# lijun9250lj/video-steganography-PCAMV

Measured on AMD Instinct MI355X. Metric: 1080p macroblocks/s (embed on), higher is better.
Workload: dtype u8

## Files before the change

### video-steganography-pcamv_amd/csrc/pcamv_common.h

```cpp
#ifndef PCAMV_COMMON_H
#define PCAMV_COMMON_H
#include <stddef.h>
#include <stdint.h>
#include "../../include/pcamv_gpu.h"

#ifdef PCAMV_HOST_EMU
#define PCAMV_DEV static inline
#define PCAMV_CONST static const
#else
#include <hip/hip_runtime.h>
#define PCAMV_DEV __device__ __forceinline__
#define PCAMV_CONST __device__ static const
#endif

#define PCAMV_PAD 32
#define PCAMV_CPAD 16
#define PCAMV_LSW 28
#define PCAMV_LROW 32
#define PCAMV_LSTRIPS(stride) (((stride) + PCAMV_LSW - 1) / PCAMV_LSW + 1)
#define PCAMV_LSTRIP_OF(x) (((uint32_t)(x) * 18725u) >> 19)
#define PCAMV_COST_MAX (1 << 28)
#define PCAMV_COST_MV_LEN (4 * 4 * 2048 + 1)
#define PCAMV_COST_MV_CENTRE (2 * 4 * 2048)
#define SCAN8_0 (4 + 1 * 8)
// ... 59 lines not shown
PCAMV_DEV int scan8_of(int idx) { return SCAN8_0 + blk_x_of(idx) + 8 * blk_y_of(idx); }
PCAMV_DEV int clip3i(int v, int lo, int hi) { return v < lo ? lo : v > hi ? hi : v; }
PCAMV_DEV int iabs(int v) { return v < 0 ? -v : v; }
PCAMV_DEV int imin(int a, int b) { return a < b ? a : b; }
PCAMV_DEV int imax(int a, int b) { return a > b ? a : b; }
PCAMV_DEV int median3i(int a, int b, int c) { return imax(imin(a, b), imin(imax(a, b), c)); }
PCAMV_DEV int size_ue_of(unsigned v) { int n = 0; for (v++; v > 1; v >>= 1) n++; return 2 * n + 1; }
enum { I4_V, I4_H, I4_DC, I4_DDL, I4_DDR, I4_VR, I4_HD, I4_VL, I4_HU, I4_DC_LEFT, I4_DC_TOP, I4_DC_128 };

struct MBLocal {
    uint8_t fenc[24 * 16];
    int16_t cmv[48][2];
    int8_t cref[48];
    int16_t pskip_mv[2];
    int16_t mvr_own[2];
    int mb_x, mb_y, mb_xy;
    int mv_min[2], mv_max[2], mv_min_spel[2], mv_max_spel[2], mv_min_fpel[2], mv_max_fpel[2];
    int neighbour, type_left, type_top, type_topleft, type_topright;
    int i_type, i_partition;
    uint8_t sub_part[4];
    int b_skip_mc, cbp_luma, cbp_chroma;
    int nnz_mask;
    uint32_t cxy[64];
    int ccost[192];
    int slots[16];
    uint8_t recb[24 * 16];
    uint8_t recb0[24 * 16];
    uint8_t pred[24 * 16];
    union {
        struct {
            int16_t coef[24][16];
            int16_t cdc[2][4];
            int blk_nz[24], blk_score[24];
            int red[64];
        };
        uint8_t pred4[4][24 * 16];
    };
    int mvc16[9][2];
    int nbc[12];
    uint32_t win[(4 * 480 + 2 * 192) / 4];
    int win_x0, win_y0, win_cx0, win_cy0;
    uint8_t ib_top[3][28];
    uint8_t ib_left[3][16];
    uint8_t nzc[48];
    int16_t cmvd[48][2];
    int8_t i4mode[48];
    int cbp_left, cbp_top;
    int b_fast_intra, fenc_satd_sum, fenc_sa8d_sum;
    uint8_t snap_pred[24 * 16];
    uint8_t snap_nzc[48];
    int16_t snap_cmvd[48][2];
    int snap_cbp_luma, snap_cbp_chroma, snap_nnz_mask;
    int snap_part, snap_cost;
#ifdef PCAMV_SEARCH_CALL
    const struct FrameDev *fdesc;
    int me_tmp[10];
    int mvc_tmp[9][2];
#endif
};
#define PCAMV_PASS2_LDS ((int)offsetof(MBLocal, coef))
static_assert(offsetof(MBLocal, pred) + sizeof(((MBLocal *)0)->pred) == offsetof(MBLocal, coef), "pred must end at the second pass' LDS cut");
static_assert(offsetof(MBLocal, fenc) < PCAMV_PASS2_LDS && offsetof(MBLocal, cmv) < PCAMV_PASS2_LDS && offsetof(MBLocal, cref) < PCAMV_PASS2_LDS &&
              offsetof(MBLocal, nnz_mask) < PCAMV_PASS2_LDS && offsetof(MBLocal, slots) + sizeof(((MBLocal *)0)->slots) <= PCAMV_PASS2_LDS &&
              offsetof(MBLocal, ccost) + sizeof(((MBLocal *)0)->ccost) <= PCAMV_PASS2_LDS, "a field the second pass uses lies beyond its LDS");
static_assert(offsetof(MBLocal, ccost) == offsetof(MBLocal, cxy) + sizeof(((MBLocal *)0)->cxy), "cxy and ccost must be contiguous (cab_residual_walk)");
static_assert(offsetof(MBLocal, recb0) == offsetof(MBLocal, recb) + 384 && offsetof(MBLocal, pred) == offsetof(MBLocal, recb) + 768 &&
              offsetof(MBLocal, coef) == offsetof(MBLocal, recb) + 1152, "recb, recb0, pred, the union must be contiguous in this order (TESA_SLOT, L_IFD)");
#define PCAMV_CHAIN_NZ 464
#define PCAMV_CHAIN_MVD 488
#define PCAMV_CHAIN_BYTES 576
#define L_CAB(L, k) ((uint8_t *)(L)->win + 464 * (k))
#define PCAMV_CAB_USED 276
#define L_CABT(L) ((uint8_t *)(L)->win + 464)
#define L_CABK(L) ((uint8_t *)(L)->win + 464 + PCAMV_CAB_USED)
#define L_CTAB(L) ((L)->win + 256)
#define L_IFD(L) ((uint8_t *)(L)->recb)
#define IFD(L, x, y) (L_IFD(L)[((y) + 1) * 32 + (x) + 4])
PCAMV_DEV int scan8_all_of(int idx)
{
    if (idx < 16) return scan8_of(idx);
    if (idx < 24) return 1 + ((idx - 16) & 1) + 8 * (1 + (((idx - 16) >> 1) & 1) + 3 * ((idx - 16) >> 2));
    return 4 + (idx - 24) + 5 * 8;
}

#define TESA_MAX_RANGE 16
#define TESA_REGION_A ((int)((3 * 24 * 16 + 4 * 24 * 16) / 4))
#define TESA_SLOT(L, i) ((i) < TESA_REGION_A ? (uint32_t *)((uint8_t *)(L) + offsetof(MBLocal, recb)) + (i) : (L)->win + ((i) - TESA_REGION_A))
#define TESA_PACK(sad, ry, rx) ((uint32_t)(sad) << 12 | (uint32_t)(ry) << 6 | (uint32_t)(rx))
#define TESA_SAD(e) ((int)((e) >> 12))
#define NB_LEFT 1
#define NB_TOP 2
#define NB_TOPRIGHT 4
#define NB_TOPLEFT 8

#define CAND_PACK(X, Y) ((uint32_t)(uint16_t)(X) | ((uint32_t)(uint16_t)(Y) << 16))
#define CAND_NONE 0x80008000u
#define CAND_X(c) ((int)(int16_t)(L->cxy[c] & 0xffffu))
#define CAND_Y(c) ((int)(int16_t)(L->cxy[c] >> 16))
#define EV_SATD 1
#define EV_CHROMA 2
#define EV_FPEL 4
#define EV_NOMV 8
#define EV_PROBE 16
#define EV_WIN 32
#define EV_SRC4 64
#define WIN_LW 24
#define WIN_LH 20
#define WIN_LP (WIN_LW * WIN_LH)
#define WIN_CW 16
#define WIN_CH 12
#define WIN_CP (WIN_CW * WIN_CH)
struct EvalRes { int cost, idx; };
#ifdef PCAMV_HOST_EMU
// ... 57 lines not shown
```

### video-steganography-pcamv_amd/csrc/pcamv_kernels.hip.h

```cpp
#ifndef PCAMV_KERNELS_HIP_H
#define PCAMV_KERNELS_HIP_H
#include "pcamv_common.h"
#include "pcamv_prims_gpu.h"
#include "pcamv_mbkernels.h"
#include "stc_mats.h"
#include "pcamv_stc_extract.h"

#if !defined(PCAMV_TESA_TU) && !defined(PCAMV_RD_TU)
#define PCAMV_MAIN_TU 1
#endif

#ifdef PCAMV_MAIN_TU
static __global__ void __launch_bounds__(256) k_chroma_pad(const FrameDev *__restrict__ Fs)
{
    const FrameDev &F = Fs[blockIdx.z >> 1];
    const int pl = blockIdx.z & 1;
    const uint8_t *__restrict__ src = F.raw[1 + pl];
    uint8_t *__restrict__ dst = F.chroma_base[pl];
    const int w = F.w >> 1, h = F.h >> 1, cstride = F.cstride, clines = F.clines;
    const int x = 4 * (blockIdx.x * blockDim.x + threadIdx.x), y = blockIdx.y;
    if (x >= cstride || y >= clines) return;
    const uint8_t *rowp = src + (size_t)clip3i(y - PCAMV_CPAD, 0, h - 1) * w;
    const int gx = x - PCAMV_CPAD;
    uint32_t v;
// ... 643 lines not shown
        const unsigned long long t_f = PROF_T();
        __builtin_amdgcn_fence(__ATOMIC_ACQUIRE, "wavefront");
        const int g = (int)((item - 1u) >> 16), xy = (int)((item - 1u) & 0xffffu);
        const FrameDev F = Fs[g];
        const int y = xy / fl.mb_w, x = xy - y * fl.mb_w;
        if (MODE == 0) PROF_ADD(15, t_f);
        PROF_ADD(MODE ? 13 : 0, t_pop);
        const unsigned long long t_s = PROF_T();
#ifdef PCAMV_SEARCH_CALL
        if (MODE == 0 && lane == 0) L.fdesc = Fs + g;
#endif
        if (MODE == 0 && (TESA & 4)) { if (!mbk_search_spec<TESA>(F, &L, Ap, x, y, fl, g, item)) break; }
        else if (MODE == 0) mbk_search<TESA>(F, &L, Ap, x, y);
        else {
            const int x0 = fl.unit * x, n = imin(fl.unit, F.mb_w - x0);
            p2_unit_load(F, Up, x0, y, n);
            for (int k = 0; k < n; k++) {
                P2Pre pre;
                pre.r = &Up->rec[k]; pre.base = Up->car_base[k]; pre.any_flip = Up->mbflip[k]; pre.nnz1 = Up->nnz1[k]; pre.drain = k > 0;
                if (mbk_pass2(F, &L, x0 + k, y, 0, &pre)) p2_put_mb(Up, &L, k);
                mbk_deblock_unit(F, Up, &L, k, x0 + k, y);
            }
            p2_unit_store(F, Up, x0, y, n);
        }
        PROF_ADD(MODE ? 14 : 1, t_s);
        const unsigned long long t_p = PROF_T();
        asm volatile("s_waitcnt vmcnt(0)" ::: "memory");
        if (MODE == 0 && (TESA & 4)) { }
        else if (lane == 0 && fl.raster) {
            if (xy + 1 < fl.n_mb) flow_done_one(fl, g & (fl.nq - 1), g * fl.n_mb + xy + 1, item + 1u);
        } else if (lane == 0) {
            const int base = g * fl.n_mb, q = g & (fl.nq - 1);
            if (x + 1 < fl.mb_w) flow_done_one(fl, q, base + xy + 1, item + 1u);
            if (y + 1 < fl.mb_h) {
                if (x >= 1) flow_done_one(fl, q, base + xy + fl.mb_w - 1, item + (unsigned)fl.mb_w - 1u);
                if (x == fl.mb_w - 1) flow_done_one(fl, q, base + xy + fl.mb_w, item + (unsigned)fl.mb_w);
            }
        }
        PROF_ADD(MODE ? 15 : 2, t_p);
        const unsigned long long t_r = PROF_T();
        if (MODE == 0 && fl.fused) {
            if (!fl.raster) {
                if (lane == 0) ticket = __hip_atomic_fetch_add(&fl.ctr[FLOW_HEAD(home)], 1u, RLX_AGENT);
                have_ticket = true;
            }
            mbk_rca_encode(F, &L, Ap, xy, 1, (TESA & 2) && F.b_mbrd);
        }
        PROF_ADD(3, t_r);
        if (MODE == 0) PROF_ADD(4, t_pop);
    }
    PROF_FLUSH();
}

#ifdef PCAMV_MAIN_TU
static __global__ void __launch_bounds__(64, PCAMV_FLOW_OCC) k_analyse_flow(const FrameDev *__restrict__ Fs, FlowDev fl)
{
    __shared__ MBLocal L;
    __shared__ Analysis A;
    flow_loop<0, 0>(Fs, fl, L, &A, nullptr);
}
#endif
#ifdef PCAMV_TESA_TU
static __global__ void __launch_bounds__(64, PCAMV_FLOW_OCC) k_analyse_flow_tesa(const FrameDev *__restrict__ Fs, FlowDev fl)
{
    __shared__ MBLocal L;
    __shared__ Analysis A;
    flow_loop<0, 1>(Fs, fl, L, &A, nullptr);
}
#endif
void pcamv_launch_flow_tesa(unsigned waves, hipStream_t st, const FrameDev *dF, const FlowDev &fl);
#ifdef PCAMV_RD_TU
#ifndef PCAMV_RD_OCC
#define PCAMV_RD_OCC 4
#endif
#ifndef PCAMV_RD_VARIANT
#define PCAMV_RD_VARIANT 2
#endif
static __global__ void __launch_bounds__(64, PCAMV_RD_OCC) k_analyse_flow_rd(const FrameDev *__restrict__ Fs, FlowDev fl)
{
    __shared__ MBLocal L;
    __shared__ Analysis A;
    flow_loop<0, PCAMV_RD_VARIANT>(Fs, fl, L, &A, nullptr);
}
#endif

#ifndef PCAMV_PASS2_OCC
#define PCAMV_PASS2_OCC 4
#endif
#ifdef PCAMV_MAIN_TU
static __global__ void __launch_bounds__(64, PCAMV_PASS2_OCC) k_pass2_deblock_flow(const FrameDev *__restrict__ Fs, FlowDev fl)
{
    __shared__ __attribute__((aligned(16))) uint8_t Lraw[PCAMV_PASS2_LDS];
    __shared__ __attribute__((aligned(16))) P2Unit U;
    flow_loop<1, 0>(Fs, fl, *reinterpret_cast<MBLocal *>(Lraw), nullptr, &U);
}
#endif

#ifdef PCAMV_MAIN_TU
static __global__ void __launch_bounds__(64) k_block_costs(const FrameDev *__restrict__ Fs, const int *__restrict__ req, int *__restrict__ out)
{
    __shared__ MBLocal L;
    const FrameDev F = Fs[0];
    const int *r = req + 8 * blockIdx.x;
    L.mb_x = r[0]; L.mb_y = r[1]; L.mb_xy = r[1] * F.mb_w + r[0];
    prim_load_fenc(F, &L);
    PCAMV_WAVE_SYNC();
// ... 490 lines not shown
```

### video-steganography-pcamv_amd/csrc/pcamv_logic.h

```cpp
#ifndef PCAMV_LOGIC_H
#define PCAMV_LOGIC_H
#include "pcamv_common.h"

PCAMV_DEV void cache_mv_set(MBLocal *L, int x, int y, int w, int h, int mvx, int mvy)
{
    PCAMV_WAVE_SYNC();
    FOR_CAND(i, w * h) {
        int j = i / w, k = i - j * w, idx = SCAN8_0 + x + k + 8 * (y + j);
        L->cmv[idx][0] = (int16_t)mvx; L->cmv[idx][1] = (int16_t)mvy;
    }
    PCAMV_WAVE_SYNC();
}
PCAMV_DEV void cache_ref_set(MBLocal *L, int x, int y, int w, int h, int ref)
{
    PCAMV_WAVE_SYNC();
    FOR_CAND(i, w * h) { int j = i / w, k = i - j * w; L->cref[SCAN8_0 + x + k + 8 * (y + j)] = (int8_t)ref; }
    PCAMV_WAVE_SYNC();
}

PCAMV_DEV void predict_from3(int ref, int refa, int refb, int refc, const int16_t *a, const int16_t *b, const int16_t *c, int mvp[2])
{
    int cnt = (refa == ref) + (refb == ref) + (refc == ref);
    if (cnt > 1) { mvp[0] = median3i(a[0], b[0], c[0]); mvp[1] = median3i(a[1], b[1], c[1]); }
    else if (cnt == 1) {
// ... 632 lines not shown
{
    const int amvd = iabs(L->cmvd[scan8_of(idx) - 1][l]) + iabs(L->cmvd[scan8_of(idx) - 8][l]);
    const int a = iabs(mvd), base = l ? 47 : 40;
    prim_cb_dec(L, C, base + (amvd > 2) + (amvd > 32), a != 0);
    if (!a) return;
    for (int i = 1; i < imin(a, 4); i++) prim_cb_dec(L, C, base + i + 2, 1);
    if (a >= 4) prim_cb_run(L, C, base + 6, imin(a, 9) - 4, a < 9);
    else prim_cb_dec(L, C, base + a + 2, 0);
    if (a >= 9) prim_cb_bypass(C, (size_ue_of((unsigned)(a - 9 + 7)) - 3) << 8);
    prim_cb_bypass(C, 256);
}
PCAMV_DEV void cb_mvd(MBLocal *L, CabWalk &C, int idx, int width, int height)
{
    int mvp[2];
    predict_mv(L, idx, width, mvp);
    const int dx = L->cmv[scan8_of(idx)][0] - mvp[0], dy = L->cmv[scan8_of(idx)][1] - mvp[1];
    cb_mvd_cpn(L, C, idx, 0, dx);
    cb_mvd_cpn(L, C, idx, 1, dy);
    for (int j = 0; j < height; j++)
        for (int i = 0; i < width; i++) { L->cmvd[scan8_of(idx) + i + 8 * j][0] = (int16_t)dx; L->cmvd[scan8_of(idx) + i + 8 * j][1] = (int16_t)dy; }
}
PCAMV_DEV void cabac_mb_header(const FrameDev &F, MBLocal *L, CabWalk &C)
{
    prim_cb_dec(L, C, 14, 0);
    if (L->i_type == PCAMV_P_8x8 || L->i_partition == PCAMV_D_16x16) { prim_cb_dec(L, C, 15, 0); prim_cb_dec(L, C, 16, L->i_type == PCAMV_P_8x8); }
    else { prim_cb_dec(L, C, 15, 1); prim_cb_dec(L, C, 17, L->i_partition == PCAMV_D_16x8); }
    if (L->i_type == PCAMV_P_8x8) {
        for (int i = 0; i < 4; i++) {
            const int sp = L->sub_part[i];
            prim_cb_dec(L, C, 21, sp == PCAMV_D_L0_8x8);
            if (sp != PCAMV_D_L0_8x8) { prim_cb_dec(L, C, 22, sp != PCAMV_D_L0_8x4); if (sp != PCAMV_D_L0_8x4) prim_cb_dec(L, C, 23, sp == PCAMV_D_L0_4x8); }
        }
        for (int i = 0; i < 4; i++)
            switch (L->sub_part[i]) {
            case PCAMV_D_L0_8x8: cb_mvd(L, C, 4 * i, 2, 2); break;
            case PCAMV_D_L0_8x4: cb_mvd(L, C, 4 * i, 2, 1); cb_mvd(L, C, 4 * i + 2, 2, 1); break;
            case PCAMV_D_L0_4x8: cb_mvd(L, C, 4 * i, 1, 2); cb_mvd(L, C, 4 * i + 1, 1, 2); break;
            default: for (int k = 0; k < 4; k++) cb_mvd(L, C, 4 * i + k, 1, 1); break;
            }
    } else if (L->i_partition == PCAMV_D_16x16) cb_mvd(L, C, 0, 4, 4);
    else if (L->i_partition == PCAMV_D_16x8) { cb_mvd(L, C, 0, 4, 2); cb_mvd(L, C, 8, 4, 2); }
    else { cb_mvd(L, C, 0, 2, 4); cb_mvd(L, C, 4, 2, 4); }
    const int cbp = L->cbp_luma, cl = L->cbp_left, ct = L->cbp_top;
    prim_cb_dec(L, C, 76 - ((cl >> 1) & 1) - ((ct >> 1) & 2), cbp & 1);
    prim_cb_dec(L, C, 76 - (cbp & 1) - ((ct >> 2) & 2), (cbp >> 1) & 1);
    prim_cb_dec(L, C, 76 - ((cl >> 3) & 1) - ((cbp << 1) & 2), (cbp >> 2) & 1);
    prim_cb_dec(L, C, 76 - ((cbp >> 2) & 1) - (cbp & 2), (cbp >> 3) & 1);
    const int ca = cl & 0x30, cb = ct & 0x30;
    prim_cb_dec(L, C, 77 + ((ca && cl != -1) ? 1 : 0) + ((cb && ct != -1) ? 2 : 0), L->cbp_chroma != 0);
    if (L->cbp_chroma) prim_cb_dec(L, C, 77 + 4 + (ca == 0x20) + 2 * (cb == 0x20), L->cbp_chroma > 1);
    if (L->cbp_luma | L->cbp_chroma) prim_cb_dec(L, C, 60, 0);
    (void)F;
}
PCAMV_DEV int rd_cost_mb(const FrameDev &F, MBLocal *L)
{
    L->b_skip_mc = 0;
    const unsigned long long t_e = PROF_T();
    mb_encode(F, L, 0, 1);
    PROF_ADD(18, t_e);
    const unsigned long long t_s = PROF_T();
    const int ssd = prim_ssd_mb(F, L);
    PROF_ADD(19, t_s);
    int bits;
    if (F.b_cabac) {
        const unsigned long long t_h = PROF_T();
        CabWalk C;
        prim_cab_begin(L, C, 1);
        cabac_mb_header(F, L, C);
        PROF_ADD(20, t_h);
        const unsigned long long t_r = PROF_T();
        prim_cab_residual(F, L, C, 0);
        const int f8 = prim_cab_end(L, C, 0);
        PROF_ADD(21, t_r);
        bits = (int)(((unsigned long long)(unsigned)f8 * (unsigned long long)F.lambda2 + 32768ull) >> 16);
    } else
        bits = (int)((unsigned)prim_cavlc_mb(F, L) * (unsigned)F.lambda2 + 128u) >> 8;
    return ssd + bits;
}
PCAMV_DEV unsigned long long rd_cost_part8(const FrameDev &F, MBLocal *L, int i8)
{
    L->b_skip_mc = 0;
    L->cbp_luma = 0;
    prim_encode_p8x8(F, L, i8);
    const unsigned long long ssd = (unsigned long long)(unsigned)prim_ssd_part8(F, L, i8);
    unsigned long long bits;
    if (F.b_cabac) {
        CabWalk C;
        prim_cab_begin(L, C, 1);
        switch (L->sub_part[i8]) {
        case PCAMV_D_L0_8x8: cb_mvd(L, C, 4 * i8, 2, 2); break;
        case PCAMV_D_L0_8x4: cb_mvd(L, C, 4 * i8, 2, 1); cb_mvd(L, C, 4 * i8 + 2, 2, 1); break;
        case PCAMV_D_L0_4x8: cb_mvd(L, C, 4 * i8, 1, 2); cb_mvd(L, C, 4 * i8 + 1, 1, 2); break;
        default: for (int k = 0; k < 4; k++) cb_mvd(L, C, 4 * i8 + k, 1, 1); break;
        }
        prim_cab_residual_part(F, L, C, i8);
        const int f8 = prim_cab_end(L, C, 0);
        bits = ((unsigned long long)(unsigned)f8 * (unsigned long long)F.lambda2 + 128ull) >> 8;
    } else
        bits = (unsigned long long)(unsigned)prim_cavlc_part8(F, L, i8) * (unsigned long long)F.lambda2;
#if defined(PCAMV_TRACE) && !defined(PCAMV_HOST_EMU)
    if (F.trace && L->mb_xy == F.trace_mb && LANE() == 0) {
        int k = F.trace[0];
        if (k < 4000) { int *t = F.trace + 1 + 8 * k; t[0] = -1; t[1] = i8; t[2] = L->sub_part[i8]; t[3] = (int)ssd; t[4] = (int)bits; t[5] = L->cbp_luma; t[6] = L->cmv[scan8_of(4 * i8)][0]; t[7] = L->cmv[scan8_of(4 * i8)][1]; F.trace[0] = k + 1; }
    }
#endif
    return (ssd << 8) + bits;
}
PCAMV_DEV int rd_trial(const FrameDev &F, MBLocal *L, int counts)
{
    const int cost = rd_cost_mb(F, L);
    if (counts && cost < L->snap_cost) { L->snap_cost = cost; L->snap_part = L->i_partition; prim_rd_keep(F, L); }
    return cost;
}
template <int TESA>
PCAMV_DEV void analyse_p_rd(const FrameDev &F, MBLocal *L, struct Analysis *a, int i_satd)
{
    const int thresh = i_satd * 5 / 4;
    L->i_type = PCAMV_P_L0;
    if (a->rd16x16 == PCAMV_COST_MAX && a->me16x16.cost <= i_satd * 3 / 2) { L->i_partition = PCAMV_D_16x16; update_cache(L, a); a->rd16x16 = rd_trial(F, L, 1); }
    a->me16x16.cost = a->rd16x16;
    if (a->cost16x8 <= thresh) { L->i_partition = PCAMV_D_16x8; update_cache(L, a); a->cost16x8 = rd_trial(F, L, 1); } else a->cost16x8 = PCAMV_COST_MAX;
    if (a->cost8x16 <= thresh) { L->i_partition = PCAMV_D_8x16; update_cache(L, a); a->cost8x16 = rd_trial(F, L, 1); } else a->cost8x16 = PCAMV_COST_MAX;
    if (a->cost8x8 <= thresh) {
        L->i_type = PCAMV_P_8x8; L->i_partition = PCAMV_D_8x8;
        unsigned inter_now = F.inter;
#ifndef PCAMV_HOST_EMU
        asm volatile("" : "+s"(inter_now));
#endif
        if ((TESA & 8) && (inter_now & PCAMV_ANALYSE_PSUB8x8)) {
            for (int i = 0; i < 4; i++) {
                const int c0 = a->cost4x4[i], c1 = a->cost8x4[i], c2 = a->cost4x8[i], c3 = a->me8x8[i].cost;
                const int th = imin(imin(c0, c1), imin(c2, c3)) * 5 / 4;
                int btype = PCAMV_D_L0_8x8;
                unsigned long long bcost = ~0ull;
                for (int subtype = PCAMV_D_L0_4x4; subtype <= PCAMV_D_L0_8x8; subtype++) {
                    const int c = subtype == 0 ? c0 : subtype == 1 ? c1 : subtype == 2 ? c2 : c3;
                    if (c > th || (subtype == PCAMV_D_L0_8x8 && bcost == ~0ull)) continue;
                    L->sub_part[i] = (uint8_t)subtype;
                    cache_mv_p8x8(L, a, i);
                    const unsigned long long cost = rd_cost_part8(F, L, i);
                    if (cost < bcost) { bcost = cost; btype = subtype; }
                }
                L->sub_part[i] = (uint8_t)btype;
                cache_mv_p8x8(L, a, i);
            }
        } else update_cache(L, a);
        a->cost8x8 = rd_trial(F, L, F.embed);
    } else a->cost8x8 = PCAMV_COST_MAX;
}
PCAMV_DEV void entropy_commit(const FrameDev &F, MBLocal *L, int walked)
{
    const int skip = L->i_type == PCAMV_P_SKIP;
    if (F.b_cabac) {
        CabWalk C;
        prim_cab_begin(L, C, 0);
        prim_cb_dec(L, C, 11 + (L->type_left >= 0 && L->type_left != PCAMV_P_SKIP) + (L->type_top >= 0 && L->type_top != PCAMV_P_SKIP), skip);
        if (!skip && !walked) { cabac_mb_header(F, L, C); prim_cab_residual(F, L, C, 1); }
        prim_cab_end(L, C, 1);
    } else if (!skip && !walked) prim_cavlc_mb(F, L);
    prim_rd_commit(F, L, skip);
}

template <int TESA>
PCAMV_DEV int analyse_p16x16(const FrameDev &F, MBLocal *L, Analysis *a, int b_try_pskip)
// ... 180 lines not shown
    if (!b_1_neighbor) cost_opt = (int)(beta1 * (float)cost_opt);
    else if (b_error_pos) cost_opt = (int)(beta2 * (float)cost_opt);
    me->mv[0] = bmx; me->mv[1] = bmy;
    update_cache(L, a);
    return cost_opt;
}

PCAMV_DEV int carrier_slots(int i_type, int i_partition, const uint8_t *sub, int used, int slots[16])
{
    int n = 0;
    if (!used) return 0;
    if (i_type == PCAMV_P_8x8) {
        for (int i = 0; i < 4; i++)
            switch (sub[i]) {
            case PCAMV_D_L0_8x8: slots[n++] = i * 4; break;
            case PCAMV_D_L0_4x8: slots[n++] = i * 4; slots[n++] = i * 4 + 1; break;
            case PCAMV_D_L0_8x4: slots[n++] = i * 4; slots[n++] = i * 4 + 2; break;
            default: for (int j = 0; j < 4; j++) slots[n++] = i * 4 + j; break;
            }
    } else if (i_type == PCAMV_P_L0) {
        if (i_partition == PCAMV_D_16x16) slots[n++] = 0;
        else if (i_partition == PCAMV_D_8x16) { slots[n++] = 0; slots[n++] = 4; }
        else if (i_partition == PCAMV_D_16x8) { slots[n++] = 0; slots[n++] = 8; }
    }
    return n;
}

PCAMV_DEV int carrier_of_block(int i_type, int i_partition, const uint8_t *sub, int i)
{
    if (i_type == PCAMV_P_8x8) {
        const int i8 = i >> 2, j = i & 3;
        switch (sub[i8]) {
        case PCAMV_D_L0_8x8: return 4 * i8;
        case PCAMV_D_L0_4x8: return 4 * i8 + (j & 1);
        case PCAMV_D_L0_8x4: return 4 * i8 + (j & 2);
        default: return i;
        }
    }
    if (i_partition == PCAMV_D_8x16) return blk_x_of(i) < 2 ? 0 : 4;
    if (i_partition == PCAMV_D_16x8) return blk_y_of(i) < 2 ? 0 : 8;
    return 0;
}

template <int TESA>
PCAMV_DEV int analyse_s16(const FrameDev &F, MBLocal *L, Analysis *a)
{
    int b_skip = 0, b_try_pskip = 0;
    for (int i = 0; i < 4; i++) L->sub_part[i] = PCAMV_D_L0_8x8;
    L->i_partition = PCAMV_D_16x16;
    a->rd16x16 = a->cost8x8 = a->cost16x8 = a->cost8x16 = PCAMV_COST_MAX;
    for (int i = 0; i < 4; i++) a->cost4x4[i] = a->cost8x4[i] = a->cost4x8[i] = PCAMV_COST_MAX;
    a->rd16_early = 0;
    L->snap_part = -1; L->snap_cost = PCAMV_COST_MAX;
    if (F.b_fast_pskip) {
        if (F.subme >= 3) b_try_pskip = 1;
        else if (L->type_left == PCAMV_P_SKIP || L->type_top == PCAMV_P_SKIP || L->type_topleft == PCAMV_P_SKIP || L->type_topright == PCAMV_P_SKIP)
            b_skip = probe_pskip(F, L);
    }
    if (b_skip) { L->i_type = PCAMV_P_SKIP; L->i_partition = PCAMV_D_16x16; return 1; }
    return analyse_p16x16<TESA>(F, L, a, b_try_pskip);
}
template <int TESA>
PCAMV_DEV void analyse_s_rest(const FrameDev &F, MBLocal *L, Analysis *a)
{
    int i_cost;
    const unsigned flags = F.inter;
    int i_type = PCAMV_P_L0, i_partition = PCAMV_D_16x16;
    const unsigned long long t_b = PROF_T();
    if (flags & PCAMV_ANALYSE_PSUB16x16) analyse_p8x8<TESA>(F, L, a);
    PROF_ADD(7, t_b);
    const unsigned long long t_c = PROF_T();
    i_cost = a->me16x16.cost;
    if ((flags & PCAMV_ANALYSE_PSUB16x16) && a->cost8x8 < a->me16x16.cost) {
        if (flags & PCAMV_ANALYSE_PSUB8x8) {
            i_type = PCAMV_P_8x8; i_partition = PCAMV_D_8x8; i_cost = a->cost8x8;
            for (int i = 0; i < 4; i++) {
                analyse_sub8x8<TESA>(F, L, a, i, PIX_4x4);
                if (a->cost4x4[i] < a->me8x8[i].cost) {
                    int c8 = a->cost4x4[i];
                    L->sub_part[i] = PCAMV_D_L0_4x4;
                    analyse_sub8x8<TESA>(F, L, a, i, PIX_8x4);
                    if (a->cost8x4[i] < c8) { c8 = a->cost8x4[i]; L->sub_part[i] = PCAMV_D_L0_8x4; }
                    analyse_sub8x8<TESA>(F, L, a, i, PIX_4x8);
                    if (a->cost4x8[i] < c8) { c8 = a->cost4x8[i]; L->sub_part[i] = PCAMV_D_L0_4x8; }
                    i_cost += c8 - a->me8x8[i].cost;
                }
                cache_mv_p8x8(L, a, i);
            }
            a->cost8x8 = i_cost;
        }
    }
    if ((flags & PCAMV_ANALYSE_PSUB16x16) && a->cost8x8 < a->me16x16.cost + a->me8x8[1].cost_mv + a->me8x8[2].cost_mv) {
        analyse_p16x8<TESA>(F, L, a);
        if (a->cost16x8 < i_cost) { i_cost = a->cost16x8; i_type = PCAMV_P_L0; i_partition = PCAMV_D_16x8; }
        analyse_p8x16<TESA>(F, L, a);
        if (a->cost8x16 < i_cost) { i_cost = a->cost8x16; i_type = PCAMV_P_L0; i_partition = PCAMV_D_8x16; }
    }
    L->i_partition = i_partition;
    a->sel_type = i_type; a->sel_part = i_partition; a->sel_cost = i_cost;
    PROF_ADD(8, t_c);
}
template <int TESA>
PCAMV_DEV void analyse_decide(const FrameDev &F, MBLocal *L, Analysis *a)
{
    int i_type = a->sel_type, i_partition = a->sel_part, i_cost = a->sel_cost;
    const unsigned long long t_d = PROF_T();
// ... 86 lines not shown
```

### video-steganography-pcamv_amd/csrc/pcamv_prims_rd_gpu.h

```cpp
#ifndef PCAMV_PRIMS_RD_GPU_H
#define PCAMV_PRIMS_RD_GPU_H

__device__ __forceinline__ uint32_t rep4(int v) { return (uint32_t)(v & 255) * 0x01010101u; }
__device__ __forceinline__ int bsum4(uint32_t v) { return (int)__builtin_amdgcn_sad_u8(v, 0u, 0u); }

struct MbFetch { uint32_t fy, fc, role, s0, s1, s2, t0, t1, t2, t3; int b0, b1; };
__device__ __forceinline__ void prim_mb_fetch(const FrameDev &F, int mb_x_, int mb_y_, int nb_, int rd_, MbFetch &P)
{
    const int mb_x = rfl(mb_x_), mb_y = rfl(mb_y_), nb = rfl(nb_), rd = rfl(rd_);
    const int lane = LANE();
    const int xy = mb_y * F.mb_w + mb_x, top = xy - F.mb_w;
    { const int row = lane >> 2, c4 = lane & 3;
      P.fy = *(const uint32_t *)(F.fenc[0] + (size_t)(mb_y * 16 + row) * F.w + mb_x * 16 + c4 * 4); }
    P.fc = 0;
    if (lane < 32) {
        const int plane = lane >> 4, row = (lane & 15) >> 1, c4 = lane & 1;
        P.fc = *(const uint32_t *)((plane ? F.fenc[2] : F.fenc[1]) + (size_t)(mb_y * 8 + row) * (F.w >> 1) + mb_x * 8 + c4 * 4);
    }
    P.role = 0; P.b0 = P.b1 = 0; P.s0 = P.s1 = P.s2 = P.t0 = P.t1 = P.t2 = P.t3 = 0;
    if (!rd) return;
    {
        const int k8 = lane & 7, l8 = (lane >> 3) & 1, ok8 = lane < 16 && (l8 ? (nb & NB_LEFT) : (nb & NB_TOP));
        const int k32 = (lane - 16) & 7, l32 = k32 >> 2, ok32 = lane >= 16 && lane < 24 && (l32 ? (nb & NB_LEFT) : (nb & NB_TOP));
        const int ok16 = (lane == 24 && (nb & NB_TOP)) || (lane == 25 && (nb & NB_LEFT));
// ... 452 lines not shown
__device__ __forceinline__ void cabq_push_run(unsigned long long &q, int &n, int owner, int ones, int zero)
{
    const bool me = LANE() == owner;
    q |= me ? ((1ull << ones) - 1ull) << n : 0ull;
    n += me ? ones + zero : 0;
}
__device__ __forceinline__ int cabq_resolve(const uint32_t *T, int &st, unsigned long long &q, int &n)
{
    int bits = 0;
    while (__builtin_amdgcn_ballot_w64(n > 0)) {
        if (n > 0) {
            const uint32_t w = T[2 * st + (int)(q & 1ull)];
            bits += (int)(w >> 8); st = (int)(w & 255u);
            q >>= 1; n--;
        }
    }
    q = 0;
    return bits;
}
__device__ __forceinline__ int cab_hdr_ctx(int lane) { return lane >= 24 && lane < 36 ? lane + 49 : lane; }
__device__ __forceinline__ int cab_hdr_lane(int ctx) { return ctx < 64 ? ctx : ctx - 49; }
__device__ __forceinline__ void prim_cab_begin(MBLocal *L, CabWalk &C, int trial_)
{
    PCAMV_WAVE_SYNC();
    const int lane = LANE();
    const uint8_t *S = L_CAB(L, 0);
    if (rfl(trial_)) {
        const uint32_t *s = (const uint32_t *)S; uint32_t *d = (uint32_t *)L_CABT(L);
        d[lane] = s[lane]; if (lane < PCAMV_CAB_USED / 4 - 64) d[64 + lane] = s[64 + lane];
    }
    C.s = S[cab_hdr_ctx(lane)]; C.bits = 0; C.vbits = 0;
    C.q = 0; C.n = 0; C.tot = 0;
}
__device__ __forceinline__ void prim_cab_flush(MBLocal *L, CabWalk &C)
{
    C.vbits += cabq_resolve(L_CTAB(L), C.s, C.q, C.n);
    C.tot = 0;
}
__device__ __forceinline__ void prim_cb_dec(MBLocal *L, CabWalk &C, int ctx_, int b_)
{
    const int ctx = rfl(ctx_), b = rfl(b_);
    if (rfl(C.tot) >= 48) prim_cab_flush(L, C);
    cabq_push(C.q, C.n, cab_hdr_lane(ctx), b);
    C.tot++;
}
__device__ __forceinline__ void prim_cb_run(MBLocal *L, CabWalk &C, int ctx_, int ones_, int zero_)
{
    const int ctx = rfl(ctx_), ones = rfl(ones_), zero = rfl(zero_);
    if (rfl(C.tot) >= 48) prim_cab_flush(L, C);
    cabq_push_run(C.q, C.n, cab_hdr_lane(ctx), ones, zero);
    C.tot += ones + zero;
}
__device__ __forceinline__ void prim_cb_bypass(CabWalk &C, int f8) { C.bits += rfl(f8); }
__device__ __forceinline__ int prim_cab_end(MBLocal *L, CabWalk &C, int commit_)
{
    const int lane = LANE();
    const uint32_t *T = L_CTAB(L);
    C.vbits += cabq_resolve(T, C.s, C.q, C.n);
    {
        uint8_t *S = rfl(commit_) ? L_CAB(L, 0) : L_CABT(L);
        S[cab_hdr_ctx(lane)] = (uint8_t)C.s;
    }
    const int total = rfl(C.bits) + wave_sum_all(C.vbits);
    PCAMV_WAVE_SYNC();
    return total;
}
struct CabBits { int bits, vbits; };
#ifdef PCAMV_RESIDUAL_CALL
#define PCAMV_RESIDUAL_FN static __device__ __noinline__
#else
#define PCAMV_RESIDUAL_FN __device__ __forceinline__
#endif
PCAMV_RESIDUAL_FN CabBits cab_residual_walk(MBLocal *L, int commit_, int part_)
{
    CabBits out = {0, 0};
    const int commit = rfl(commit_);
    const int lane = LANE();
    PCAMV_WAVE_SYNC();
    const int cbp_luma = rfl(L->cbp_luma), cbp_chroma = rfl(L->cbp_chroma);
    if (!(cbp_luma | cbp_chroma)) return out;
    uint8_t *S = L_CAB(L, 0);
    uint8_t *D = commit ? S : L_CABT(L);
    const uint32_t *T = L_CTAB(L);
    int bits = 0, sbits = 0;
    const unsigned long long t_1 = PROF_T();
    const int part = rfl(part_);
    const bool coded = part >= 0 ? (lane < 16 ? (lane >> 2) == part && ((cbp_luma >> part) & 1) != 0 : lane < 24 ? ((lane - 16) & 3) == part : false)
                     : lane < 16 ? ((cbp_luma >> (lane >> 2)) & 1) != 0 : lane < 24 ? (cbp_chroma & 2) != 0 : lane < 26 ? (cbp_chroma & 3) != 0 : false;
    const int idx = lane < 24 ? lane : lane < 26 ? 25 + (lane - 24) : 0;
    const int count = lane < 16 ? 16 : lane < 24 ? 15 : 4;
    int flag = 0, inc = 0;
    unsigned nzm = 0, gt1 = 0, nib0 = 0, nib1 = 0;
    if (coded) {
        const int p8 = scan8_all_of(idx);
        flag = L->nzc[p8] != 0;
        if (lane >= 24) {
            const int cl = L->cbp_left, ct = L->cbp_top, k = lane - 24;
            inc = (cl != -1 ? (cl >> (9 + k)) & 1 : 0) + 2 * (ct != -1 ? (ct >> (9 + k)) & 1 : 0);
        } else inc = ((L->nzc[p8 - 1] & 0x7f) != 0) + 2 * ((L->nzc[p8 - 8] & 0x7f) != 0);
        if (flag) {
            const uint32_t *w = lane < 24 ? (const uint32_t *)L->coef[lane] : (const uint32_t *)L->cdc[lane - 24];
            const int nw = lane < 24 ? 8 : 2, sh = (lane >= 16 && lane < 24) ? 1 : 0;
            unsigned nzr = 0, g1r = 0;
            unsigned long long nib = 0;
#pragma unroll
            for (int j = 0; j < 8; j++) {
// ... 269 lines not shown
    else if (is_c) { if (nz) idct4x4_add(dst, d); L->nzc[scan8_all_of(lane)] = (uint8_t)nz; }
    const unsigned long long km = __ballot(is_l && keep);
    L->cbp_luma = (L->cbp_luma & ~(1 << i8)) | (km ? 1 << i8 : 0);
    L->cbp_chroma = 2;
    PCAMV_WAVE_SYNC();
}
__device__ __forceinline__ int prim_ssd_part8(const FrameDev &F, MBLocal *L, int i8_)
{
    const int i8 = rfl(i8_);
    PCAMV_WAVE_SYNC();
    const int lane = LANE();
    const bool is_l = lane < 16 && (lane >> 2) == i8, is_c = lane >= 16 && lane < 24 && ((lane - 16) & 3) == i8;
    int v = 0;
    if (is_l || is_c) {
        const int ch = (lane - 16) >> 2, ci = (lane - 16) & 3;
        const int px = lane < 16 ? 4 * blk_x_of(lane) : ch * 8 + (ci & 1) * 4, py = lane < 16 ? 4 * blk_y_of(lane) : 16 + (ci >> 1) * 4;
#pragma unroll
        for (int k = 0; k < 4; k++) {
            const uint32_t e = lds4(L->fenc + (py + k) * 16 + px), p = lds4(L->pred + (py + k) * 16 + px);
#pragma unroll
            for (int x = 0; x < 4; x++) { const int dd = (int)((e >> (8 * x)) & 255) - (int)((p >> (8 * x)) & 255); v += mul24s(dd, dd); }
        }
    }
    int ssd = wave_sum_all(v);
    if (F.psy_rd) {
        int s4, dc, s8, f4, fdc, f8;
        had_lane_sums(L->pred, lane, &s4, &dc, &s8);
        had_lane_sums(L->fenc, lane, &f4, &fdc, &f8);
        int fs = (f4 >> 1) - (fdc >> 1);
        if (!is_l) { s4 = 0; dc = 0; s8 = 0; fs = 0; fdc = 0; f8 = 0; }
        s4 = group_sum(s4, 16); dc = group_sum(dc, 16); s8 = group_sum(s8, 16); fs = group_sum(fs, 16); fdc = group_sum(fdc, 16); f8 = group_sum(f8, 16);
        const int S4 = __builtin_amdgcn_readlane(s4, 0), DC = __builtin_amdgcn_readlane(dc, 0), S8 = __builtin_amdgcn_readlane(s8, 0);
        const int FS = __builtin_amdgcn_readlane(fs, 0), FDC = __builtin_amdgcn_readlane(fdc, 0), F8 = __builtin_amdgcn_readlane(f8, 0);
        const int sum4 = (S4 - DC) >> 1, sum8 = (S8 - DC) >> 2, fsa8d = ((F8 + 2) >> 2) - (FDC >> 2);
        const int satd = (iabs(sum4 - FS) + iabs(sum8 - fsa8d)) >> 1;
        ssd += (satd * F.psy_rd * F.lambda + 128) >> 8;
    }
    PCAMV_WAVE_SYNC();
    return ssd;
}

__device__ __forceinline__ void prim_rd_keep(const FrameDev &F, MBLocal *L)
{
    PCAMV_WAVE_SYNC();
    const int lane = LANE();
    { const uint32_t *s = (const uint32_t *)L->pred; uint32_t *d = (uint32_t *)L->snap_pred; d[lane] = s[lane]; if (lane < 32) d[64 + lane] = s[64 + lane]; }
    if (lane < 12) ((uint32_t *)L->snap_nzc)[lane] = ((const uint32_t *)L->nzc)[lane];
    if (lane < 48) ((uint32_t *)L->snap_cmvd)[lane] = ((const uint32_t *)L->cmvd)[lane];
    if (F.b_cabac) {
        const uint32_t *s = (const uint32_t *)L_CABT(L); uint32_t *d = (uint32_t *)L_CABK(L);
        d[lane] = s[lane]; if (lane < PCAMV_CAB_USED / 4 - 64) d[64 + lane] = s[64 + lane];
    }
    if (lane == 0) { L->snap_cbp_luma = L->cbp_luma; L->snap_cbp_chroma = L->cbp_chroma; L->snap_nnz_mask = L->nnz_mask; }
    PCAMV_WAVE_SYNC();
}
__device__ __forceinline__ void prim_rd_restore(const FrameDev &F, MBLocal *L)
{
    PCAMV_WAVE_SYNC();
    const int lane = LANE();
    { const uint32_t *s = (const uint32_t *)L->snap_pred; uint32_t *d = (uint32_t *)L->pred; d[lane] = s[lane]; if (lane < 32) d[64 + lane] = s[64 + lane]; }
    if (lane < 12) ((uint32_t *)L->nzc)[lane] = ((const uint32_t *)L->snap_nzc)[lane];
    if (lane < 48) ((uint32_t *)L->cmvd)[lane] = ((const uint32_t *)L->snap_cmvd)[lane];
    if (F.b_cabac) {
        const uint32_t *s = (const uint32_t *)L_CABK(L); uint32_t *d = (uint32_t *)L_CAB(L, 0);
        d[lane] = s[lane]; if (lane < PCAMV_CAB_USED / 4 - 64) d[64 + lane] = s[64 + lane];
    }
    if (lane == 0) { L->cbp_luma = L->snap_cbp_luma; L->cbp_chroma = L->snap_cbp_chroma; L->nnz_mask = L->snap_nnz_mask; }
    PCAMV_WAVE_SYNC();
}
__device__ __forceinline__ void prim_rd_commit(const FrameDev &F, MBLocal *L, int skip_)
{
    const int skip = rfl(skip_);
    const int lane = LANE();
    const int xy = L->mb_xy;
    PCAMV_WAVE_SYNC();
    if (lane < 16) {
        const int k = lane & 7, is_right = lane >> 3;
        const int blk = is_right ? (k < 4 ? (k == 0 ? 5 : k == 1 ? 7 : k == 2 ? 13 : 15) : 17 + 2 * (k - 4)) : (k < 4 ? (k == 0 ? 10 : k == 1 ? 11 : k == 2 ? 14 : 15) : k < 6 ? 18 + (k - 4) : 22 + (k - 6));
        NB_ST8(&F.nb_nz[xy * 16 + lane], skip ? 0 : L->nzc[scan8_all_of(blk)]);
    } else if (lane < 24) {
        const int k = lane - 16, pos = k < 4 ? SCAN8_0 + k + 8 * 3 : SCAN8_0 + 3 + 8 * (k - 4);
        NB_ST32(&F.nb_mvd[(xy * 8 + k) * 2], skip ? 0u : ((const uint32_t *)L->cmvd)[pos]);
    } else if (lane == 24) {
        const int cbp = skip ? 0 : ((F.b_cabac ? (L->nzc[scan8_all_of(25)] << 9 | L->nzc[scan8_all_of(26)] << 10) : 0) | L->cbp_chroma << 4 | L->cbp_luma);
        NB_ST16(&F.nb_cbp[xy], cbp);
    }
    if (F.b_cabac) {
        const uint32_t *src = (const uint32_t *)L_CAB(L, 0);
        NB_ST32((uint32_t *)F.cabac + lane, src[lane]);
        if (lane < 52) NB_ST32((uint32_t *)F.cabac + 64 + lane, src[64 + lane]);
        if (F.dbg_hash && lane == 0) {
            uint32_t h = 2166136261u;
            for (int i = 0; i < 460; i++) h = (h ^ L_CAB(L, 0)[i]) * 16777619u;
            F.dbg_hash[xy] = h;
        }
    }
    if (F.inter & PCAMV_ANALYSE_PSUB8x8) {
        uint32_t *dst = (uint32_t *)F.cabac + PCAMV_CHAIN_NZ / 4;
        if (lane < 6) {
            uint32_t w = 0;
#pragma unroll
            for (int k = 0; k < 4; k++) w |= (uint32_t)(skip ? 0 : L->nzc[scan8_all_of(4 * lane + k)]) << (8 * k);
            NB_ST32(dst + lane, w);
        } else if (lane < 22) NB_ST32(dst + lane, ((const uint32_t *)L->cmvd)[scan8_of(lane - 6)]);
    }
    PCAMV_WAVE_SYNC();
}
#endif
// ... 1 lines not shown
```

Baseline: 23.27 million.

## Reuse residual SSD and CABAC residual bits across RD trials with identical motion

When a rate-distortion trial has the same per-4x4 motion vectors as the currently kept best candidate, it skips mb_encode, the SSD computation and the CABAC residual walk. Instead it restores the snapshot nzc/cbp state and adds the cached residual bit count to a freshly coded header. This removes redundant encoding work for partition trials that converge to the same motion. The cost is extra LDS for snapshot motion vectors and a per-trial comparison, and CABAC context state after the residual may differ slightly from a full re-encode.

```diff
diff --git a/video-steganography-pcamv_amd/csrc/pcamv_common.h b/video-steganography-pcamv_amd/csrc/pcamv_common.h
--- a/video-steganography-pcamv_amd/csrc/pcamv_common.h
+++ b/video-steganography-pcamv_amd/csrc/pcamv_common.h
@@ -135,6 +135,12 @@
     int16_t snap_cmvd[48][2];
     int snap_cbp_luma, snap_cbp_chroma, snap_nnz_mask;
     int snap_part, snap_cost;
+    uint32_t snap_mv[16];
+    int snap_ssd, snap_f8r;
+#if defined(PCAMV_PROF)
+    uint32_t prof_mv[4][16];
+    int prof_ntrial;
+#endif
 #ifdef PCAMV_SEARCH_CALL
     const struct FrameDev *fdesc;
     int me_tmp[10];
@@ -142,6 +148,7 @@
 #endif
 };
 #define PCAMV_PASS2_LDS ((int)offsetof(MBLocal, coef))
+#define PCAMV_WAVE_LDS_MAX 10240
 static_assert(offsetof(MBLocal, pred) + sizeof(((MBLocal *)0)->pred) == offsetof(MBLocal, coef), "pred must end at the second pass' LDS cut");
 static_assert(offsetof(MBLocal, fenc) < PCAMV_PASS2_LDS && offsetof(MBLocal, cmv) < PCAMV_PASS2_LDS && offsetof(MBLocal, cref) < PCAMV_PASS2_LDS &&
               offsetof(MBLocal, nnz_mask) < PCAMV_PASS2_LDS && offsetof(MBLocal, slots) + sizeof(((MBLocal *)0)->slots) <= PCAMV_PASS2_LDS &&
diff --git a/video-steganography-pcamv_amd/csrc/pcamv_kernels.hip.h b/video-steganography-pcamv_amd/csrc/pcamv_kernels.hip.h
--- a/video-steganography-pcamv_amd/csrc/pcamv_kernels.hip.h
+++ b/video-steganography-pcamv_amd/csrc/pcamv_kernels.hip.h
@@ -719,6 +719,9 @@
     PROF_FLUSH();
 }
 
+#ifndef PCAMV_PROF
+static_assert(sizeof(MBLocal) + sizeof(Analysis) <= PCAMV_WAVE_LDS_MAX, "the analysis kernels' LDS per wave (MBLocal + Analysis) no longer allows 16 waves per CU");
+#endif
 #ifdef PCAMV_MAIN_TU
 static __global__ void __launch_bounds__(64, PCAMV_FLOW_OCC) k_analyse_flow(const FrameDev *__restrict__ Fs, FlowDev fl)
 {
diff --git a/video-steganography-pcamv_amd/csrc/pcamv_logic.h b/video-steganography-pcamv_amd/csrc/pcamv_logic.h
--- a/video-steganography-pcamv_amd/csrc/pcamv_logic.h
+++ b/video-steganography-pcamv_amd/csrc/pcamv_logic.h
@@ -708,15 +708,21 @@
     if (L->cbp_luma | L->cbp_chroma) prim_cb_dec(L, C, 60, 0);
     (void)F;
 }
-PCAMV_DEV int rd_cost_mb(const FrameDev &F, MBLocal *L)
+struct RdParts { int ssd, f8r; };
+PCAMV_DEV int rd_cost_mb(const FrameDev &F, MBLocal *L, RdParts *parts, int reuse)
 {
     L->b_skip_mc = 0;
-    const unsigned long long t_e = PROF_T();
-    mb_encode(F, L, 0, 1);
-    PROF_ADD(18, t_e);
-    const unsigned long long t_s = PROF_T();
-    const int ssd = prim_ssd_mb(F, L);
-    PROF_ADD(19, t_s);
+    if (!reuse) {
+        const unsigned long long t_e = PROF_T();
+        mb_encode(F, L, 0, 1);
+        PROF_ADD(18, t_e);
+        const unsigned long long t_s = PROF_T();
+        parts->ssd = prim_ssd_mb(F, L); parts->f8r = 0;
+        PROF_ADD(19, t_s);
+    }
+#ifndef PCAMV_HOST_EMU
+    else prim_rd_reuse_begin(L);
+#endif
     int bits;
     if (F.b_cabac) {
         const unsigned long long t_h = PROF_T();
@@ -725,13 +731,24 @@
         cabac_mb_header(F, L, C);
         PROF_ADD(20, t_h);
         const unsigned long long t_r = PROF_T();
+        int f8;
+#if !defined(PCAMV_HOST_EMU) && !defined(PCAMV_RD_NO_REUSE)
+        if (reuse) f8 = prim_cab_end(L, C, 0) + parts->f8r;
+        else {
+            const int f8h = prim_cab_bits_so_far(L, C);
+            prim_cab_residual(F, L, C, 0);
+            f8 = prim_cab_end(L, C, 0);
+            parts->f8r = f8 - f8h;
+        }
+#else
         prim_cab_residual(F, L, C, 0);
-        const int f8 = prim_cab_end(L, C, 0);
+        f8 = prim_cab_end(L, C, 0);
+#endif
         PROF_ADD(21, t_r);
         bits = (int)(((unsigned long long)(unsigned)f8 * (unsigned long long)F.lambda2 + 32768ull) >> 16);
     } else
         bits = (int)((unsigned)prim_cavlc_mb(F, L) * (unsigned)F.lambda2 + 128u) >> 8;
-    return ssd + bits;
+    return parts->ssd + bits;
 }
 PCAMV_DEV unsigned long long rd_cost_part8(const FrameDev &F, MBLocal *L, int i8)
 {
@@ -764,8 +781,25 @@
 }
 PCAMV_DEV int rd_trial(const FrameDev &F, MBLocal *L, int counts)
 {
-    const int cost = rd_cost_mb(F, L);
-    if (counts && cost < L->snap_cost) { L->snap_cost = cost; L->snap_part = L->i_partition; prim_rd_keep(F, L); }
+    RdParts parts;
+    int reuse = 0;
+#if !defined(PCAMV_HOST_EMU) && (!defined(PCAMV_RD_NO_REUSE) || defined(PCAMV_PROF))
+    const bool same = rfl(L->snap_part) >= 0 && prim_rd_same_motion(L);
+#ifdef PCAMV_PROF
+    prim_rd_prof_trial(L, same);
+#endif
+#ifndef PCAMV_RD_NO_REUSE
+    if (same && F.b_cabac) { reuse = 1; parts.ssd = L->snap_ssd; parts.f8r = L->snap_f8r; }
+#endif
+#endif
+    const int cost = rd_cost_mb(F, L, &parts, reuse);
+    if (counts && cost < L->snap_cost) {
+        L->snap_cost = cost; L->snap_part = L->i_partition;
+#ifndef PCAMV_HOST_EMU
+        if (reuse) { PROF_CNT(46, 1); prim_rd_keep_header(L); } else
+#endif
+        { L->snap_ssd = parts.ssd; L->snap_f8r = parts.f8r; prim_rd_keep(F, L); }
+    }
     return cost;
 }
 template <int TESA>
@@ -1052,6 +1086,9 @@
     for (int i = 0; i < 4; i++) a->cost4x4[i] = a->cost8x4[i] = a->cost4x8[i] = PCAMV_COST_MAX;
     a->rd16_early = 0;
     L->snap_part = -1; L->snap_cost = PCAMV_COST_MAX;
+#if defined(PCAMV_PROF) && !defined(PCAMV_HOST_EMU)
+    L->prof_ntrial = 0;
+#endif
     if (F.b_fast_pskip) {
         if (F.subme >= 3) b_try_pskip = 1;
         else if (L->type_left == PCAMV_P_SKIP || L->type_top == PCAMV_P_SKIP || L->type_topleft == PCAMV_P_SKIP || L->type_topright == PCAMV_P_SKIP)
diff --git a/video-steganography-pcamv_amd/csrc/pcamv_prims_rd_gpu.h b/video-steganography-pcamv_amd/csrc/pcamv_prims_rd_gpu.h
--- a/video-steganography-pcamv_amd/csrc/pcamv_prims_rd_gpu.h
+++ b/video-steganography-pcamv_amd/csrc/pcamv_prims_rd_gpu.h
@@ -528,6 +528,11 @@
     C.tot += ones + zero;
 }
 __device__ __forceinline__ void prim_cb_bypass(CabWalk &C, int f8) { C.bits += rfl(f8); }
+__device__ __forceinline__ int prim_cab_bits_so_far(MBLocal *L, CabWalk &C)
+{
+    prim_cab_flush(L, C);
+    return rfl(C.bits) + wave_sum_all(C.vbits);
+}
 __device__ __forceinline__ int prim_cab_end(MBLocal *L, CabWalk &C, int commit_)
 {
     const int lane = LANE();
@@ -903,8 +908,46 @@
         d[lane] = s[lane]; if (lane < PCAMV_CAB_USED / 4 - 64) d[64 + lane] = s[64 + lane];
     }
     if (lane == 0) { L->snap_cbp_luma = L->cbp_luma; L->snap_cbp_chroma = L->cbp_chroma; L->snap_nnz_mask = L->nnz_mask; }
-    PCAMV_WAVE_SYNC();
-}
+    if (lane < 16) L->snap_mv[lane] = ((const uint32_t *)L->cmv)[scan8_of(lane)];
+    PCAMV_WAVE_SYNC();
+}
+__device__ __forceinline__ bool prim_rd_same_motion(MBLocal *L)
+{
+    PCAMV_WAVE_SYNC();
+    const int lane = LANE();
+    const bool differs = lane < 16 && ((const uint32_t *)L->cmv)[scan8_of(lane)] != L->snap_mv[lane];
+    return __builtin_amdgcn_ballot_w64(differs) == 0ull;
+}
+__device__ __forceinline__ void prim_rd_reuse_begin(MBLocal *L)
+{
+    PCAMV_WAVE_SYNC();
+    const int lane = LANE();
+    if (lane < 12) ((uint32_t *)L->nzc)[lane] = ((const uint32_t *)L->snap_nzc)[lane];
+    if (lane == 0) { L->cbp_luma = L->snap_cbp_luma; L->cbp_chroma = L->snap_cbp_chroma; L->nnz_mask = L->snap_nnz_mask; }
+    PCAMV_WAVE_SYNC();
+}
+__device__ __forceinline__ void prim_rd_keep_header(MBLocal *L)
+{
+    PCAMV_WAVE_SYNC();
+    const int lane = LANE();
+    if (lane < 48) ((uint32_t *)L->snap_cmvd)[lane] = ((const uint32_t *)L->cmvd)[lane];
+    L_CABK(L)[cab_hdr_ctx(lane)] = L_CABT(L)[cab_hdr_ctx(lane)];
+    PCAMV_WAVE_SYNC();
+}
+#ifdef PCAMV_PROF
+__device__ __forceinline__ void prim_rd_prof_trial(MBLocal *L, bool same_kept)
+{
+    PCAMV_WAVE_SYNC();
+    const int lane = LANE(), n = rfl(L->prof_ntrial);
+    const uint32_t mv = lane < 16 ? ((const uint32_t *)L->cmv)[scan8_of(lane)] : 0u;
+    int same_other = 0;
+    for (int k = 0; k < n; k++) same_other |= __builtin_amdgcn_ballot_w64(lane < 16 && mv != L->prof_mv[k][lane]) == 0ull;
+    PROF_CNT(43, 1); PROF_CNT(44, same_kept ? 1 : 0); PROF_CNT(45, !same_kept && same_other ? 1 : 0);
+    if (lane < 16 && n < 4) L->prof_mv[n][lane] = mv;
+    if (lane == 0) L->prof_ntrial = n + 1;
+    PCAMV_WAVE_SYNC();
+}
+#endif
 __device__ __forceinline__ void prim_rd_restore(const FrameDev &F, MBLocal *L)
 {
     PCAMV_WAVE_SYNC();
```

Result: faster. 24.79 million, median of 6 (+6.5%).
